# dzatulin/llama-fastapi-k8s-gpu

Measured on AMD Instinct MI355X. Metric: output tokens/sec + p50 /response latency, Llama-3-8B Q4_K_M at 1/2/4/8 MI355X, higher is better.
Workload: dtype q4_k_m weights; f16 (batched decode and prompt prefill MFMA, tile16 copies) / int8 (single-row GEMV) activations; fp32 accumulate

## Files before the change

csrc/bindings_hip.cpp:

```cpp
#include <pybind11/functional.h>
#include <pybind11/numpy.h>
#include <pybind11/pybind11.h>
#include <pybind11/stl.h>

#include <array>
#include <rccl/rccl.h>

#include "bind_scheduler.h"
#include "kernels/kernels.h"
#include "runtime/engine.h"
#include "runtime/repack.h"

namespace py = pybind11;
using namespace lfk;

template <class T>
static T* P(uintptr_t p) { return reinterpret_cast<T*>(p); }
static hipStream_t S(uintptr_t s) { return reinterpret_cast<hipStream_t>(s); }

static void hip_ok(const char* what) {
  hipError_t e = hipGetLastError();
  if (e != hipSuccess) throw std::runtime_error(std::string(what) + ": " + hipGetErrorString(e));
}

// ... 305 lines not shown
  });

  m.def("bprep", [](uintptr_t x, int ldx, bool swiglu, uintptr_t norm, float eps, int K, int B, uintptr_t xh, int ldh,
                    uintptr_t stream, uintptr_t zero, int zero_n, int swiglu_group) {
    BPrepArgs a;
    a.swiglu_group = swiglu_group;
    a.x = P<float>(x); a.ldx = ldx; a.swiglu = swiglu; a.norm_w = P<float>(norm); a.eps = eps; a.K = K; a.B = B;
    a.xh = P<__half>(xh); a.ldh = ldh; a.zero = P<float>(zero); a.zero_n = zero_n;
    bprep(a, S(stream));
    hip_ok("bprep");
  }, py::arg("x"), py::arg("ldx"), py::arg("swiglu"), py::arg("norm"), py::arg("eps"), py::arg("K"), py::arg("B"),
     py::arg("xh"), py::arg("ldh"), py::arg("stream"), py::arg("zero") = 0, py::arg("zero_n") = 0,
     py::arg("swiglu_group") = 32);
  m.def("bmm", [](uintptr_t w, int type, int rows, int K, uintptr_t xh, int ldh, uintptr_t out, int ldo, int B,
                  uintptr_t stream, int debug, uintptr_t h_out, int ldh_out, uintptr_t xf, int ldxf,
                  uintptr_t norm, float eps, bool store_out, uintptr_t dbg_clk, int tr) {
    BmmArgs a;
    a.debug = debug;
    a.tr = tr;
    a.dbg_clk = P<long long>(dbg_clk);
    a.w = make_qmat(P<void>(w), type, rows, K);
    a.xh = P<__half>(xh); a.ldh = ldh; a.out = P<float>(out); a.ldo = ldo; a.n_out = rows; a.B = B;
    if (h_out) {
      a.swiglu_epi = true; a.h_out = P<__half>(h_out); a.ldh_out = ldh_out;
    }
    if (xf) {
      a.xf = P<float>(xf); a.ldxf = ldxf; a.norm_w = P<float>(norm); a.eps = eps;
    }
    a.store_out = store_out;
    bmm(a, S(stream));
    hip_ok("bmm");
  }, py::arg("w"), py::arg("type"), py::arg("rows"), py::arg("K"), py::arg("xh"), py::arg("ldh"), py::arg("out"),
     py::arg("ldo"), py::arg("B"), py::arg("stream"), py::arg("debug") = 0, py::arg("h_out") = 0,
     py::arg("ldh_out") = 0, py::arg("xf") = 0, py::arg("ldxf") = 0, py::arg("norm") = 0, py::arg("eps") = 1e-5f,
     py::arg("store_out") = false, py::arg("dbg_clk") = 0, py::arg("tr") = -1);
  m.def("chain_layout", []() { return std::make_tuple(kChainStride, kChainXcds, kChainInts); });
  m.def("bmm_ffn_chain", [](uintptr_t wg, int tg, int F, int K, uintptr_t xh, uintptr_t xf, uintptr_t norm, float eps,
                            uintptr_t wd, int td, uintptr_t hout, uintptr_t out, int B, uintptr_t cnt,
                            uintptr_t stream, int tr) {
    BmmArgs gu, dn;
    dn.tr = tr;
    gu.w = make_qmat(P<void>(wg), tg, 2 * F, K);
    gu.xh = P<__half>(xh); gu.ldh = K; gu.n_out = 2 * F; gu.B = B;
    gu.swiglu_epi = true; gu.h_out = P<__half>(hout); gu.ldh_out = F;
    if (xf) {
      gu.xf = P<float>(xf); gu.ldxf = K; gu.norm_w = P<float>(norm); gu.eps = eps;
    }
    dn.w = make_qmat(P<void>(wd), td, K, F);
    dn.xh = P<__half>(hout); dn.ldh = F; dn.out = P<float>(out); dn.ldo = K; dn.n_out = K; dn.B = B;
    if (!bmm_ffn_chain_supported(gu, dn)) throw std::runtime_error("bmm_ffn_chain: unsupported shapes");
    bmm_ffn_chain(gu, dn, P<int>(cnt), nullptr, S(stream));
    hip_ok("bmm_ffn_chain");
  }, py::arg("wg"), py::arg("tg"), py::arg("F"), py::arg("K"), py::arg("xh"), py::arg("xf"), py::arg("norm"),
     py::arg("eps"), py::arg("wd"), py::arg("td"), py::arg("hout"), py::arg("out"), py::arg("B"), py::arg("cnt"),
     py::arg("stream"), py::arg("tr") = -1);
  m.def("bmm_wo_ffn_chain", [](uintptr_t wo, int to, int Kwo, uintptr_t xa, uintptr_t wg, int tg, int F, int K,
                               uintptr_t norm, float eps, uintptr_t wd, int td, uintptr_t xh, uintptr_t hout,
                               uintptr_t resid, int B, uintptr_t cnt, uintptr_t stream, int tr) {
    BmmArgs o, gu, dn;
    o.tr = dn.tr = tr;
    o.w = make_qmat(P<void>(wo), to, K, Kwo);
    o.xh = P<__half>(xa); o.ldh = Kwo; o.out = P<float>(resid); o.ldo = K; o.n_out = K; o.B = B;
    gu.w = make_qmat(P<void>(wg), tg, 2 * F, K);
    gu.xh = P<__half>(xh); gu.ldh = K; gu.n_out = 2 * F; gu.B = B;
    gu.swiglu_epi = true; gu.h_out = P<__half>(hout); gu.ldh_out = F;
    gu.xf = P<float>(resid); gu.ldxf = K; gu.norm_w = P<float>(norm); gu.eps = eps;
    dn.w = make_qmat(P<void>(wd), td, K, F);
    dn.xh = P<__half>(hout); dn.ldh = F; dn.out = P<float>(resid); dn.ldo = K; dn.n_out = K; dn.B = B;
    if (!bmm_wo_ffn_chain_supported(o, gu, dn)) throw std::runtime_error("bmm_wo_ffn_chain: unsupported shapes");
    bmm_wo_ffn_chain(o, gu, dn, P<int>(cnt), nullptr, S(stream));
// ... 273 lines not shown
```

csrc/kernels/bmm.hip:

```cpp
#include <algorithm>
#include <cstdlib>
#include <stdexcept>

#include "gemv_dev.h"

namespace lfk {

typedef _Float16 h2_t __attribute__((ext_vector_type(2)));
typedef _Float16 h8_t __attribute__((ext_vector_type(8)));
typedef float f4_t __attribute__((ext_vector_type(4)));

__device__ __forceinline__ h2_t as_h2(unsigned v) { return __builtin_bit_cast(h2_t, v); }
__device__ __forceinline__ unsigned as_u(h2_t v) { return __builtin_bit_cast(unsigned, v); }

__device__ __forceinline__ unsigned bytes02(unsigned x) { return __builtin_amdgcn_perm(0x64646464u, x, 0x04020400u); }
__device__ __forceinline__ unsigned bytes13(unsigned x) { return __builtin_amdgcn_perm(0x64646464u, x, 0x04030401u); }

__device__ __forceinline__ unsigned deq_pair(unsigned magic_pair, h2_t bias, h2_t a, h2_t m) {
  const h2_t v = as_h2(magic_pair) - bias;
  return as_u(v * a + m);
}

struct HFrag {
  unsigned w[16];
// ... 778 lines not shown
      const float ss = wave_sum_fast(x.x * x.x + x.y * x.y + x.z * x.z + x.w * x.w);
      if (lane == 0) atomicAdd(rowss + b, ss);
    }
  }
}

template <int N>
using f32v = float __attribute__((ext_vector_type(N)));
template <int N>
using u32v = unsigned __attribute__((ext_vector_type(N)));
__device__ __forceinline__ float4 ldg4(const float* p) {
  typedef float v4 __attribute__((ext_vector_type(4)));
  const v4 t = *(const __attribute__((address_space(1))) v4*)(p);
  return make_float4(t.x, t.y, t.z, t.w);
}
__device__ __forceinline__ uint4 ldg4(const __half* p) {
  typedef unsigned v4 __attribute__((ext_vector_type(4)));
  const v4 t = *(const __attribute__((address_space(1))) v4*)(p);
  return make_uint4(t.x, t.y, t.z, t.w);
}
template <int N>
__device__ __forceinline__ void vput(f32v<N>& v, int i, float4 t) {
  v[4 * i] = t.x; v[4 * i + 1] = t.y; v[4 * i + 2] = t.z; v[4 * i + 3] = t.w;
}
template <int N>
__device__ __forceinline__ float4 vget(const f32v<N>& v, int i) {
  return make_float4(v[4 * i], v[4 * i + 1], v[4 * i + 2], v[4 * i + 3]);
}
template <int NW, bool SC1 = false, class Issue>
__device__ __forceinline__ void xfirst_norm(const BmmArgs& a, __half* xs, float* rowss, int ldx, int tid, int lane,
// ... 174 lines not shown
  }();
  return a.tr < 0 ? v : a.tr != 0;
}

template <int QT, int PD, bool SK, int NW = 8, bool MOE = false, bool XF = false, int DBG = 0, bool IL = false,
          int EPI = 0, int CR = 0, bool TR = false>
__device__ __forceinline__ void wt_body(const BmmArgs& a, const int run, const int bid, const int nblk) {
  constexpr int R = PD + 1;
  extern __shared__ __attribute__((aligned(16))) char smem[];
  float* rowss = reinterpret_cast<float*>(smem);
  __half* xs = reinterpret_cast<__half*>(smem + 256);
  {
    const int f0 = a.w.K, f1 = a.kparts, f2 = a.spp, f3 = a.n_out, f4 = a.B, f5 = a.nseg, f6 = a.debug, f7 = a.chain_role;
    const int f8 = a.ldh, f9 = a.ldxf, f10 = a.zero_n, f11 = a.ldo, f12 = a.nb1, f13 = a.tpg, f14 = a.seg_split;
    const void *p0 = a.w.base, *p1 = a.xh, *p2 = a.xf, *p3 = a.norm_w, *p4 = a.zero, *p5 = a.dbg_clk, *p6 = a.out,
               *p7 = a.chain_cnt, *p8 = a.ss_out;
    asm volatile("" ::"s"(f0), "s"(f1), "s"(f2), "s"(f3), "s"(f4), "s"(f5), "s"(f6), "s"(f7), "s"(f8), "s"(f9), "s"(f10),
                 "s"(f11), "s"(f12), "s"(f13), "s"(f14), "s"(p0), "s"(p1), "s"(p2), "s"(p3), "s"(p4), "s"(p5), "s"(p6),
                 "s"(p7), "s"(p8), "s"(nblk));
  }
  const int lane = threadIdx.x & 63, wave = wave_id(), tid = threadIdx.x;
  const int r16 = lane & 15, kq = lane >> 4;
  const int K = a.w.K, steps = K >> 8;
  const int kparts = a.kparts, kp = bid % kparts, grp = bid / kparts, G = nblk / kparts;
  const int s0 = kp * a.spp, ns = min(steps, s0 + a.spp) - s0;
  const int k0 = s0 * 256, kn = ns * 256, ldx = kn + kWtXPad;
  if (MOE && !SK && a.ew && a.steps_per_expert > 0) {
    const int e = s0 / a.steps_per_expert;
    bool any = false;
    for (int b = 0; b < a.B; ++b) any = any || a.ew[(size_t)b * a.ew_ld + e] != 0.f;
    if (!any) {
      if (a.zero) {
        float4* z = reinterpret_cast<float4*>(a.zero);
        for (int i = bid * (NW * 64) + threadIdx.x; i < (a.zero_n >> 2); i += nblk * (NW * 64))
// ... 107 lines not shown
    for (int p = 0; p < PD; ++p) load_first(buf[p], p < N);
    if constexpr (SK && !IL) pos = a.qkv.pos[col_ok ? r16 : 0];
    if (!XF && xmode == 2) lds_barrier();
  };
  if (XF && xmode == 2) lds_barrier();
  __shared__ int wo_exits;
  if (tid == 0) wo_exits = 0;
  auto wo_arrive = [&]() {
    if (!SK && (a.chain_role & kChainWoDone)) {
      asm volatile("s_waitcnt vmcnt(0)" ::: "memory");
      if (lane == 0 && atomicAdd(&wo_exits, 1) == NW - 1)
        __hip_atomic_fetch_add(a.chain_cnt + (kChainWoPart * kChainXcds + (xcc_id() & (kChainXcds - 1))) * kChainStride, 1,
                               __ATOMIC_RELAXED, __HIP_MEMORY_SCOPE_AGENT);
    }
  };
  if constexpr (DBG == 4 || DBG == 6) issue();
  else if constexpr (XF) {
    if constexpr (!SK && CR == kChainConsume) {
      issue();
      chain_wait(a, kp, tid);
      xstage_sc1<NW>(a, xs, ldx, k0, kn, tid);
    } else if constexpr (!SK && CR == kChainWaitWo) {
      issue();
      count_wait(a, kChainWoPart, a.chain_wo, tid);
      xfirst_norm<NW, true>(a, xs, rowss, ldx, tid, lane, wave, [] {});
    } else if (xmode == 2) xfirst_part_norm<NW>(a, xs, rowss, ldx, k0, kn, tid, lane, issue);
    else if (xmode == 1) xfirst_norm<NW>(a, xs, rowss, ldx, tid, lane, wave, issue);
    else xfirst_plain<NW>(a, xs, rowss, ldx, k0, kn, tid, lane, wave, issue);
  } else {
    issue();
    if (xmode == 2) stage_x_part_norm<NW>(a, xs, rowss, ldx, k0, kn, tid, lane);
    else bmm_stage_x<NW>(a, xs, rowss, ldx, k0, kn, tid, lane, wave);
  }
  if constexpr (XF) lds_barrier();
  else __syncthreads();
  if (clk && tid == 0) clk[2] = wall_clock64();
  if (!SK && (a.chain_role & kChainProduce) && tid == 0)
    __hip_atomic_fetch_add(a.chain_cnt + (kChainStagedPart * kChainXcds + (xcc_id() & (kChainXcds - 1))) * kChainStride, 1,
                           __ATOMIC_RELAXED, __HIP_MEMORY_SCOPE_AGENT);
  if (SK && a.ss_out && run == 0 && grp == 0 && tid < a.B) atomicAdd(a.ss_out + tid, rowss[tid]);
  if (N == 0) {
    wo_arrive();
    return;
  }
  if constexpr (SK && !IL) {
    pos = min(max(pos, 0), a.qkv.n_ctx - 1);
    rope_load(0);
  }
  float cs = 1.f;
  if (a.xf && !SK) {
    float t = 0.f;
#pragma unroll
    for (int w = 0; w < NW; ++w) t += rowss[(col_ok ? r16 : 0) * NW + w];
    cs = rsqrtf(t / (float)K + a.eps);
  }
  const __half* xrow = xs + (col_ok ? r16 : 0) * ldx - k0;
  f4_t acc = {0.f, 0.f, 0.f, 0.f}, acc2 = {0.f, 0.f, 0.f, 0.f};
  int ci = 0, cstep = 0;
  auto add_tr = [&](float* o, int row0, int n_out, bool atomic) {
    if (row0 + r16 < n_out) {
#pragma unroll
      for (int i = 0; i < 4; ++i) {
        const int b = 4 * kq + i;
        if (b < a.B) {
          float* p = o + (size_t)b * a.ldo + row0 + r16;
// ... 1 lines not shown
          else if (a.store_out) *p = acc[i];
          else *p += acc[i];
        }
      }
    }
  };
  auto finish = [&]() {
    acc += acc2;
    if (a.debug == 3) {
      asm volatile("" ::"v"(acc[0]), "v"(acc[1]), "v"(acc[2]), "v"(acc[3]));
      acc = f4_t{0.f, 0.f, 0.f, 0.f};
      acc2 = acc;
      return;
    }
    if constexpr (!TR) {
      if (a.xf && !SK) acc *= cs;
    }
    const int gt = tile_of(ci);
    if constexpr (SK) {
      const int sg = seg_of(gt), kind = sg == 0 ? a.qkv.kind[0] : sg == 1 ? a.qkv.kind[1] : a.qkv.kind[2];
      const int n_out = sg == 0 ? a.n_out : sg == 1 ? a.seg_rows[1] : a.seg_rows[2];
      float* o = (sg == 0 ? a.out : sg == 1 ? a.seg_out[1] : a.seg_out[2]) + (size_t)r16 * a.ldo;
      const int row0 = (gt - seg_first(sg)) * 16 + 4 * kq;
      f4_t y = acc;
      if (!IL && kind < 2) {
#pragma unroll
        for (int j = 0; j < 2; ++j) {
          y[2 * j] = acc[2 * j] * rc[j].x - acc[2 * j + 1] * rc[j].y;
          y[2 * j + 1] = acc[2 * j] * rc[j].y + acc[2 * j + 1] * rc[j].x;
        }
      }
// ... 147 lines not shown
  (void)a;
  (void)b;
}

template <int QT0, int QT1, int QT2, bool TR = false>
__global__ __launch_bounds__(512, 2) void bmm_chain3_kernel(BmmArgs a, BmmArgs b, BmmArgs c) {
  const BmmArgs* ka = (const BmmArgs*)__builtin_amdgcn_kernarg_segment_ptr();
  const int n0 = ka[0].nb1, n1 = ka[1].nb1;
  const int bid = blockIdx.x;
  if (bid < n0) wt_body<QT0, 2, false, 8, false, true, 0, true, 2, 0, TR>(ka[0], 0, bid, n0);
  else if (bid < n0 + n1) wt_body<QT1, 2, false, 8, false, true, 0, true, 1, kChainWaitWo>(ka[1], 0, bid - n0, n1);
  else wt_body<QT2, 2, false, 8, false, true, 0, true, 2, kChainConsume, TR>(ka[2], 0, bid - n0 - n1, gridDim.x - n0 - n1);
  (void)a;
  (void)b;
  (void)c;
}

static constexpr int kPrepBlock = 1024;
static constexpr int kPrepMaxVec = 8;

__global__ __launch_bounds__(kPrepBlock) void bprep_kernel(BPrepArgs a) {
  __shared__ float red[kPrepBlock / 64];
  const int b = blockIdx.x, tid = threadIdx.x;
  if (b >= a.B) {
    float4* z = reinterpret_cast<float4*>(a.zero);
    const int nzb = gridDim.x - a.B;
    for (int i = (b - a.B) * kPrepBlock + tid; i < (a.zero_n >> 2); i += nzb * kPrepBlock)
      z[i] = make_float4(0.f, 0.f, 0.f, 0.f);
    return;
  }
// ... 240 lines not shown
  if (a.ew && (a.ew_ld < 1 || (a.swiglu_epi ? a.tiles_per_expert < 1 || ((a.n_out + 15) / 16) % a.tiles_per_expert
                                            : a.steps_per_expert < 1 || (a.w.K / 256) % a.steps_per_expert)))
    throw std::runtime_error("bmm: expert routing weights need whole experts of tiles / K steps");
  if (a.ew && a.swiglu_epi && (a.n_out + 15) / 16 / a.tiles_per_expert > 64) throw std::runtime_error("bmm: <= 64 experts");
  if (a.ew && !a.swiglu_epi && (a.xf || a.qkv_epi || a.one_part))
    throw std::runtime_error("bmm: the MoE down projection runs split-K (whole-expert parts)");
  if (a.qkv_sk) {
    if (a.B > 8 || a.qkv_epi || a.swiglu_epi || a.ew || a.one_part || a.store_out || !a.qkv.pos || !a.qkv.rope ||
        a.qkv.head_dim % 2 || a.qkv.n_ctx < 1 || a.seg_split < 1 || a.seg_split > a.nseg ||
        (a.seg_split < a.nseg && !bmm_qkv_sk_supported(a.w.type, a.type2, a.type2, a.w.K, a.B)))
      throw std::runtime_error("bmm: split-K Q|K|V arguments");
    if (a.xf && (!a.norm_w || !a.ss_out || a.ldxf < a.w.K || a.ldxf % 4)) throw std::runtime_error("bmm: split-K Q|K|V norm");
  }
  if (a.ss_out && !(a.qkv_sk && a.xf)) throw std::runtime_error("bmm: ss_out needs the split-K Q|K|V norm");
  if (a.zero && (a.zero_n % 4 || reinterpret_cast<uintptr_t>(a.zero) % 16)) throw std::runtime_error("bmm: zero side job alignment");
}

void bmm(const BmmArgs& a0, hipStream_t s) {
  BmmArgs a = a0;
  bmm_check(a);
  if (a.n_out <= 0) return;
  a.w.type = t16_kernel_type(a.w.type);
  a.type2 = a.type2 ? t16_kernel_type(a.type2) : 0;
  if (a.qkv_sk && a.seg_split < a.nseg && a.type2 == a.w.type) {
    a.seg_split = a.nseg;
    a.type2 = 0;
  }
  if (a.qkv_sk) {
    const bool two = a.seg_split < a.nseg;
    const int t2 = two ? a.type2 : 0;
// ... 71 lines not shown
  if (dn.kparts > kChainWoPart) throw std::runtime_error("bmm_wo_ffn_chain: too many K parts for the counters");
  wo.chain_role = kChainWoDone; wo.chain_cnt = cnt; wo.nb1 = n0;
  gu.chain_role = kChainProduce | kChainWaitWo; gu.chain_cnt = cnt; gu.chain_tpp = 32 * dn.spp; gu.chain_wo = n0;
  gu.chain_err = err; gu.chain_poll = 8; gu.nb1 = n1;
  dn.chain_role = kChainConsume; dn.chain_cnt = cnt; dn.chain_tpp = 32 * dn.spp; dn.chain_tiles = (gu.n_out + 15) / 16;
  dn.chain_err = err; dn.chain_staged = n1; dn.chain_poll = 8;
  const dim3 grid(n0 + n1 + n2);
  const size_t lds = std::max(lds0, std::max(lds1, lds2));
  if (bmm_tr(dn)) {
    if (dn.w.type == T_Q6_K) hipLaunchKernelGGL((bmm_chain3_kernel<T_Q4_K, T_Q4_K, T_Q6_K, true>), grid, dim3(512), lds, s, wo, gu, dn);
    else hipLaunchKernelGGL((bmm_chain3_kernel<T_Q4_K, T_Q4_K, T_Q4_K, true>), grid, dim3(512), lds, s, wo, gu, dn);
  } else if (dn.w.type == T_Q6_K) hipLaunchKernelGGL((bmm_chain3_kernel<T_Q4_K, T_Q4_K, T_Q6_K>), grid, dim3(512), lds, s, wo, gu, dn);
  else hipLaunchKernelGGL((bmm_chain3_kernel<T_Q4_K, T_Q4_K, T_Q4_K>), grid, dim3(512), lds, s, wo, gu, dn);
}

bool bmm_qkv2(const BmmArgs& a0, const BmmArgs& b0, hipStream_t s) {
  if (!a0.qkv_epi || !b0.qkv_epi || a0.B != b0.B || a0.w.K != b0.w.K || a0.n_out <= 0 || b0.n_out <= 0)
    return false;
  if ((a0.xf == nullptr) != (b0.xf == nullptr)) return false;
  BmmArgs a = a0, b = b0;
  bmm_check(a);
  bmm_check(b);
  auto tiles_of = [](const BmmArgs& x) {
    int t = (x.n_out + 15) / 16;
    for (int i = 1; i < x.nseg; ++i) t += (x.seg_rows[i] + 15) / 16;
    return t;
  };
  const int steps = a.w.K / 256;
  a.spp = b.spp = steps;
  a.kparts = b.kparts = 1;
// ... 294 lines not shown
```

csrc/kernels/kernels.h:

```cpp
#pragma once
#include <hip/hip_bf16.h>
#include <hip/hip_fp16.h>
#include <hip/hip_runtime.h>

#include <cstddef>
#include <cstdint>

#include "../common.h"

namespace lfk {

struct QMat {
  const uint8_t* base = nullptr;
  int type = 0;
  int rows = 0;
  int K = 0;
  Planes P{};
  size_t expert_stride = 0;
};

QMat make_qmat(const void* base, int type, int rows, int K, size_t expert_stride = 0);

inline size_t qmat_bytes(const QMat& m) {
  const size_t R = (size_t)m.rows;
// ... 94 lines not shown
    int n_ctx = 0, head_dim = 0;
    const int* pos = nullptr;
    const int* slots = nullptr;
    const float2* rope = nullptr;
    const float* bias[3] = {nullptr, nullptr, nullptr};
  } qkv;
  bool qkv_epi = false;
  __half* h_out = nullptr;
  int ldh_out = 0;
  bool swiglu_epi = false;
  int tile_groups = 1;
  const float* xf = nullptr;
  int ldxf = 0;
  const float* norm_w = nullptr;
  float eps = 1e-5f;
  bool store_out = false;
  const float* ew = nullptr;
  int ew_ld = 0, tiles_per_expert = 0, steps_per_expert = 0;
  bool one_part = false;
  int tr = -1;
  long long* dbg_clk = nullptr;
  int nb1 = 0;
  bool qkv_sk = false;
  float* ss_out = nullptr;
  int seg_split = 1;
  int type2 = 0;
  int tpg = 8;
  float* zero = nullptr;
  int zero_n = 0;
};
bool bmm_qkv_sk_supported(int tq, int tk, int tv, int K, int B);
bool bmm_supported(int type, int K);
bool bmm_qkv_fits(int K, int B);
bool bmm_norm_fits(int K, int B);
void bmm(const BmmArgs& a, hipStream_t s);
constexpr int kChainStride = 32, kChainXcds = 8, kChainMaxParts = 16;
constexpr int kChainInts = kChainStride * kChainXcds * kChainMaxParts;
constexpr int kChainStagedPart = kChainMaxParts - 1;
constexpr int kChainWoPart = kChainMaxParts - 2;
constexpr int kChainProduce = 1, kChainConsume = 2, kChainWoDone = 4, kChainWaitWo = 8;
bool bmm_ffn_chain_supported(const BmmArgs& gu, const BmmArgs& dn);
void bmm_ffn_chain(const BmmArgs& gu, const BmmArgs& dn, int* cnt, int* err, hipStream_t s);
bool bmm_wo_ffn_chain_supported(const BmmArgs& wo, const BmmArgs& gu, const BmmArgs& dn);
void bmm_wo_ffn_chain(const BmmArgs& wo, const BmmArgs& gu, const BmmArgs& dn, int* cnt, int* err, hipStream_t s);
bool bmm_qkv2(const BmmArgs& a, const BmmArgs& b, hipStream_t s);
bool bmm_qkv_sk_defers_rope();
size_t t16_bytes(int type, int rows, int K);
int t16_format(int type);
void t16_repack(const QMat& planar, uint8_t* dst, hipStream_t s, bool swiglu = false);
struct BPrepArgs {
  const float* x = nullptr;
  int ldx = 0;
  bool swiglu = false;
  const float* norm_w = nullptr;
  float eps = 1e-5f;
  int K = 0, B = 0;
  __half* xh = nullptr;
  int ldh = 0;
  float* zero = nullptr;
// ... 215 lines not shown
```

csrc/runtime/engine.cpp:

```cpp
#include "engine.h"

#include <rccl/rccl.h>
#include <rocprofiler-sdk-roctx/roctx.h>

#include <chrono>
#include <cmath>
#include <cstdio>
#include <cstring>
#include <stdexcept>

#include "repack.h"
#include "shard.h"

namespace lfk {

#define HIPCHK(x) check((x), #x)

struct RoctxRange {
  explicit RoctxRange(const char* m) { roctxRangePushA(m); }
  ~RoctxRange() { roctxRangePop(); }
};

static double now_s() {
  return std::chrono::duration<double>(std::chrono::steady_clock::now().time_since_epoch()).count();
// ... 418 lines not shown
    chain_cnt_ = (int*)dalloc(sizeof(int) * kChainInts * hp_.n_layer);
    HIPCHK(hipMemsetAsync(chain_cnt_, 0, sizeof(int) * kChainInts * hp_.n_layer, stream_));
    HIPCHK(hipHostMalloc((void**)&chain_err_h_, sizeof(int), hipHostMallocMapped));
    *chain_err_h_ = 0;
    HIPCHK(hipHostGetDevicePointer((void**)&chain_err_, chain_err_h_, 0));
  }
  const int E = std::max(1, hp_.n_expert);
  xh_b_ = (__half*)dalloc(2ull * bmax_ * std::max({hp_.n_embd, nq_, F_l_}));
  {
    const size_t n = qkv_b_zero_n();
    qkv_b_ = (float*)dalloc(sizeof(float) * n);
    HIPCHK(hipMemsetAsync(qkv_b_, 0, sizeof(float) * n, stream_));
    ss_b_ = qkv_b_ + (size_t)bmax_ * (nq_ + 2 * nkvd_);
  }
  hh_b_ = (__half*)dalloc(2ull * bmax_ * std::max(1, F_l_) * (moe_b_ ? E : 1));
  if (moe_b_) ew_b_ = (float*)dalloc(sizeof(float) * bmax_ * E);
  auto tile = [&](const QMat& m, bool swiglu = false) {
    QMat t = m;
    uint8_t* dst = (uint8_t*)dalloc(t16_bytes(m.type, m.rows, m.K));
    t16_repack(m, dst, stream_, swiglu);
    t.base = dst;
    return t;
  };
  t_output_ = tile(output_);
  for (int l = 0; l < hp_.n_layer; ++l) {
    Layer& L = layers_[l];
    L.t_wq = tile(L.wq); L.t_wk = tile(L.wk); L.t_wv = tile(L.wv); L.t_wo = tile(L.wo);
    if (bg_ffn_) { L.t_gu = tile(L.w_gu, true); L.t_down = tile(L.w_down); }
    if (moe_b_) {
      const size_t gu1 = t16_bytes(L.gu_exps.type, L.gu_exps.rows, L.gu_exps.K);
// ... 665 lines not shown
  };
  auto tp_end = [&]() {
    if (tp_acc) p2p_->allreduce_add(tmp_b_, x_, B * d, s);
    else if (tp) allreduce_into(tmp_, x_, (size_t)B * d, s);
  };
  const size_t kv_layer = (size_t)nkv_l_ * opt_.n_ctx * hd;
  __half* kcl = kc_ + kv_layer * (l - opt_.layer_begin);
  __half* vcl = vc_ + kv_layer * (l - opt_.layer_begin);
  const bool fused = B <= kBmmMaxRows && bmm_qkv_fits(d, B);
  const bool fnorm = fused && bmm_norm_fits(d, B);
  const bool sk = qkv_sk_ && bmm_qkv_sk_supported(L.t_wq.type, L.t_wk.type, L.t_wv.type, d, B) &&
                  (!L.bqkv || bmm_qkv_sk_defers_rope());
  auto zero_qkv = [&]() {
    if (sk) HIPCHK(hipMemsetAsync(qkv_b_, 0, sizeof(float) * qkv_b_zero_n(), s));
  };
  if (sk) {
    BmmArgs a;
    a.w = L.t_wq; a.n_out = L.t_wq.rows; a.out = qkv_b_; a.ldo = ncol; a.B = B;
    a.nseg = 3;
    a.seg_base[1] = L.t_wk.base; a.seg_rows[1] = L.t_wk.rows; a.seg_out[1] = qkv_b_ + nq_;
    a.seg_base[2] = L.t_wv.base; a.seg_rows[2] = L.t_wv.rows; a.seg_out[2] = qkv_b_ + nq_ + nkvd_;
    const int tq = t16_format(L.t_wq.type), tk = t16_format(L.t_wk.type), tv = t16_format(L.t_wv.type);
    a.seg_split = tk != tq ? 1 : tv != tq ? 2 : 3;
    a.type2 = tk != tq ? tk : tv != tq ? tv : 0;
    a.qkv_sk = true;
    a.qkv.pos = bpos_; a.qkv.rope = rope_; a.qkv.head_dim = hd; a.qkv.n_ctx = opt_.n_ctx;
    a.xf = x_; a.ldxf = d; a.norm_w = L.attn_norm; a.eps = hp_.rms_eps; a.ss_out = ss_b_;
    a.dbg_clk = clk_of(l, 0);
    bmm(a, s);
  } else {
// ... 45 lines not shown
  aa.scale = 1.f / std::sqrt((float)hd);
  aa.part = attn_part_b_; aa.counters = attn_cnt_b_; aa.out = attn_;
  aa.batch = B; aa.slots = bslots_; aa.slot_stride = slot_stride_;
  aa.q_stride = nq_; aa.out_stride = nq_;
  aa.part_stride = attn_decode_workspace_floats(opt_.n_ctx, nh_l_, hd);
  aa.out_h = xh_b_; aa.out_h_stride = nq_;
  aa.out = nullptr;
  if (sk) {
    aa.qkv_raw = qkv_b_; aa.qkv_ld = ncol; aa.k_off = nq_; aa.v_off = nq_ + nkvd_;
    aa.ss = ss_b_; aa.inv_k = 1.f / (float)d; aa.eps = hp_.rms_eps;
    if (bmm_qkv_sk_defers_rope()) aa.rope_freq = rope_freq_;
    aa.qkv_bias = L.bqkv;
  }
  aa.dbg_clk = clk_of(l, 1);
  attn_decode(aa, s);
  BmmArgs wo, gu, dn;
  wo.w = L.t_wo; wo.xh = xh_b_; wo.ldh = nq_; wo.out = acc; wo.ldo = d; wo.n_out = d; wo.B = B;
  wo.dbg_clk = clk_of(l, 2);
  const bool dense_ffn = !(moe_b_ && fused) && bg_ffn_ && fused;
  if (dense_ffn) {
    if (fnorm) {
      gu.xf = x_; gu.ldxf = d; gu.norm_w = L.ffn_norm; gu.eps = hp_.rms_eps;
    }
    gu.w = L.t_gu; gu.xh = xh_b_; gu.ldh = d;
    gu.out = nullptr; gu.ldo = 0; gu.n_out = 2 * F_l_; gu.B = B;
    gu.swiglu_epi = true; gu.h_out = hh_b_; gu.ldh_out = F_l_;
    gu.dbg_clk = clk_of(l, 3);
    dn.w = L.t_down; dn.xh = hh_b_; dn.ldh = F_l_; dn.out = acc; dn.ldo = d; dn.n_out = d; dn.B = B;
    dn.dbg_clk = clk_of(l, 4);
    if (sk) {
      dn.zero = qkv_b_; dn.zero_n = (int)qkv_b_zero_n();
    }
    if (ffn_chain_ >= 2 && !tp && fnorm && B <= kBmmMaxRows && bmm_wo_ffn_chain_supported(wo, gu, dn)) {
      bmm_wo_ffn_chain(wo, gu, dn, chain_cnt_ + kChainInts * l, chain_err_, s);
      return;
    }
  }
  tp_begin();
  if (B <= kBmmMaxRows) bmm(wo, s);
  else bmm_rows(L.t_wo, xh_b_, nq_, acc, d, d, B, s, clk_of(l, 2));
  tp_end();
  if (moe_b_ && fused) {
    const int E = hp_.n_expert;
    moe_router_rows(x_, d, B, L.ffn_norm, hp_.rms_eps, reinterpret_cast<const float*>(L.router.base), d, E,
                    hp_.n_expert_used, ew_b_, E, s);
    BmmArgs a;
    if (fnorm) {
      a.xf = x_; a.ldxf = d; a.norm_w = L.ffn_norm; a.eps = hp_.rms_eps;
    } else {
      bprep_rows(x_, d, false, L.ffn_norm, d, B, nullptr, 0, s);
    }
    a.w = L.t_gu; a.xh = xh_b_; a.ldh = d;
    a.out = nullptr; a.ldo = 0; a.n_out = L.t_gu.rows; a.B = B;
    a.swiglu_epi = true; a.h_out = hh_b_; a.ldh_out = E * F_l_;
// ... 954 lines not shown
```

csrc/runtime/engine.h:

```cpp
#pragma once
#include <hip/hip_runtime.h>

#include <atomic>
#include <functional>
#include <memory>
#include <mutex>
#include <string>
#include <vector>

#include "../kernels/kernels.h"
#include "gguf.h"
#include "p2p.h"
#include "slots.h"
#include "tp_channel.h"

namespace lfk {


struct EngineOptions {
  int n_ctx = 1024;
  int n_batch = 512;
  int device = 0;
  bool use_graph = true;
  int tp_rank = 0;
// ... 269 lines not shown
  long long* step_clk_ = nullptr;
  int step_clk_layer_ = -1;
  long long* clk_of(int l, int k) const {
    return l == step_clk_layer_ && step_clk_ ? step_clk_ + (size_t)k * kStepClkBlocks * 16 : nullptr;
  }
  float* qkv_b_ = nullptr;
  float* ss_b_ = nullptr;
  bool wo_fuse_ = true;
  bool moe_route_fuse_ = true;
  int* wo_err_h_ = nullptr;
  int* wo_err_ = nullptr;
  int ffn_chain_ = 1;
  int* chain_cnt_ = nullptr;
  int* chain_err_h_ = nullptr;
  int* chain_err_ = nullptr;
  int* dec_done_ = nullptr;
  size_t qkv_b_zero_n() const { return (size_t)bmax_ * (nq_ + 2 * nkvd_) + 16; }

  std::vector<hipGraphExec_t> bgraph_;
  std::vector<hipGraphExec_t> bgraph2_;
  int launch_par_ = 0;
  int dslot_ = 0;
  std::vector<hipGraphExec_t> sgraph_, sgraph2_;
  bool last_b1_ = false;
  hipGraph_t graph_ = nullptr;
  hipGraphExec_t graph_exec_ = nullptr, graph_exec2_ = nullptr;
  void enqueue_stage_decode(hipStream_t s);
  void chain_step(const Engine* prev, const Engine* last, const std::vector<Engine*>& others);
  hipGraphExec_t chain_graph_[2] = {nullptr, nullptr};
  int chain_par_ = 0;
// ... 7 lines not shown
```

Measured before the change: 2860.

## Fuse FFN RMSNorm prep into a wave-owned Wo kernel with deferred row scale

Adds a Wo projection kernel in which each block owns a 16-column tile over the full K. It adds the residual, writes the updated residual, emits the norm-weighted f16 FFN input and per-tile partial sums of squares. The gate/up SwiGLU kernel then reads those f16 rows and reduces the partial sums to apply the RMS scale after accumulation, instead of staging and normalising fp32 rows itself. This is meant to remove the per-block norm/staging work in gate/up for small decode batches (B<=8). The cost is that Wo runs with only n_out/16 blocks and no split-K, and the activation is rounded to f16 before the scale is applied.

Result: no change. 2858 (-0.0%).

```diff
diff --git a/csrc/bindings_hip.cpp b/csrc/bindings_hip.cpp
--- a/csrc/bindings_hip.cpp
+++ b/csrc/bindings_hip.cpp
@@ -343,7 +343,7 @@
      py::arg("swiglu_group") = 32);
   m.def("bmm", [](uintptr_t w, int type, int rows, int K, uintptr_t xh, int ldh, uintptr_t out, int ldo, int B,
                   uintptr_t stream, int debug, uintptr_t h_out, int ldh_out, uintptr_t xf, int ldxf,
-                  uintptr_t norm, float eps, bool store_out, uintptr_t dbg_clk, int tr) {
+                  uintptr_t norm, float eps, bool store_out, uintptr_t dbg_clk, int tr, uintptr_t xss) {
     BmmArgs a;
     a.debug = debug;
     a.tr = tr;
@@ -356,17 +356,41 @@
     if (xf) {
       a.xf = P<float>(xf); a.ldxf = ldxf; a.norm_w = P<float>(norm); a.eps = eps;
     }
+    if (xss) {
+      a.xss = P<float>(xss); a.eps = eps;
+    }
     a.store_out = store_out;
     bmm(a, S(stream));
     hip_ok("bmm");
   }, py::arg("w"), py::arg("type"), py::arg("rows"), py::arg("K"), py::arg("xh"), py::arg("ldh"), py::arg("out"),
      py::arg("ldo"), py::arg("B"), py::arg("stream"), py::arg("debug") = 0, py::arg("h_out") = 0,
      py::arg("ldh_out") = 0, py::arg("xf") = 0, py::arg("ldxf") = 0, py::arg("norm") = 0, py::arg("eps") = 1e-5f,
-     py::arg("store_out") = false, py::arg("dbg_clk") = 0, py::arg("tr") = -1);
+     py::arg("store_out") = false, py::arg("dbg_clk") = 0, py::arg("tr") = -1, py::arg("xss") = 0);
+  m.def("bmm_wo_own", [](uintptr_t w, int type, int rows, int K, uintptr_t xh, int ldh, uintptr_t out, int ldo, int B,
+                         uintptr_t norm, uintptr_t hn, int ldhn, uintptr_t ss, uintptr_t stream, uintptr_t dbg_clk) {
+    BmmArgs a;
+    a.w = make_qmat(P<void>(w), type, rows, K);
+    a.xh = P<__half>(xh); a.ldh = ldh; a.out = P<float>(out); a.ldo = ldo; a.n_out = rows; a.B = B;
+    a.norm_w = P<float>(norm); a.h_out = P<__half>(hn); a.ldh_out = ldhn; a.ss_out = P<float>(ss);
+    a.dbg_clk = P<long long>(dbg_clk);
+    bmm_wo_own(a, S(stream));
+    hip_ok("bmm_wo_own");
+  }, py::arg("w"), py::arg("type"), py::arg("rows"), py::arg("K"), py::arg("xh"), py::arg("ldh"), py::arg("out"),
+     py::arg("ldo"), py::arg("B"), py::arg("norm"), py::arg("hn"), py::arg("ldhn"), py::arg("ss"), py::arg("stream"),
+     py::arg("dbg_clk") = 0);
+  m.def("bmm_wo_own_supported", [](int type, int rows, int K, int B) {
+    BmmArgs a;
+    __half* h = reinterpret_cast<__half*>(16);
+    float* f = reinterpret_cast<float*>(16);
+    a.w = make_qmat(nullptr, type, rows, K);
+    a.xh = h; a.ldh = K; a.out = f; a.ldo = rows; a.n_out = rows; a.B = B; a.norm_w = f; a.h_out = h; a.ldh_out = rows;
+    a.ss_out = f;
+    return bmm_wo_own_supported(a);
+  });
   m.def("chain_layout", []() { return std::make_tuple(kChainStride, kChainXcds, kChainInts); });
   m.def("bmm_ffn_chain", [](uintptr_t wg, int tg, int F, int K, uintptr_t xh, uintptr_t xf, uintptr_t norm, float eps,
                             uintptr_t wd, int td, uintptr_t hout, uintptr_t out, int B, uintptr_t cnt,
-                            uintptr_t stream, int tr) {
+                            uintptr_t stream, int tr, uintptr_t xss) {
     BmmArgs gu, dn;
     dn.tr = tr;
     gu.w = make_qmat(P<void>(wg), tg, 2 * F, K);
@@ -375,6 +399,9 @@
     if (xf) {
       gu.xf = P<float>(xf); gu.ldxf = K; gu.norm_w = P<float>(norm); gu.eps = eps;
     }
+    if (xss) {
+      gu.xss = P<float>(xss); gu.eps = eps;
+    }
     dn.w = make_qmat(P<void>(wd), td, K, F);
     dn.xh = P<__half>(hout); dn.ldh = F; dn.out = P<float>(out); dn.ldo = K; dn.n_out = K; dn.B = B;
     if (!bmm_ffn_chain_supported(gu, dn)) throw std::runtime_error("bmm_ffn_chain: unsupported shapes");
@@ -382,7 +409,7 @@
     hip_ok("bmm_ffn_chain");
   }, py::arg("wg"), py::arg("tg"), py::arg("F"), py::arg("K"), py::arg("xh"), py::arg("xf"), py::arg("norm"),
      py::arg("eps"), py::arg("wd"), py::arg("td"), py::arg("hout"), py::arg("out"), py::arg("B"), py::arg("cnt"),
-     py::arg("stream"), py::arg("tr") = -1);
+     py::arg("stream"), py::arg("tr") = -1, py::arg("xss") = 0);
   m.def("bmm_wo_ffn_chain", [](uintptr_t wo, int to, int Kwo, uintptr_t xa, uintptr_t wg, int tg, int F, int K,
                                uintptr_t norm, float eps, uintptr_t wd, int td, uintptr_t xh, uintptr_t hout,
                                uintptr_t resid, int B, uintptr_t cnt, uintptr_t stream, int tr) {
diff --git a/csrc/kernels/bmm.hip b/csrc/kernels/bmm.hip
--- a/csrc/kernels/bmm.hip
+++ b/csrc/kernels/bmm.hip
@@ -816,6 +816,7 @@
   const v4 t = *(const __attribute__((address_space(1))) v4*)(p);
   return make_float4(t.x, t.y, t.z, t.w);
 }
+__device__ __forceinline__ float ldg1(const float* p) { return *(const __attribute__((address_space(1))) float*)(p); }
 __device__ __forceinline__ uint4 ldg4(const __half* p) {
   typedef unsigned v4 __attribute__((ext_vector_type(4)));
   const v4 t = *(const __attribute__((address_space(1))) v4*)(p);
@@ -1020,10 +1021,10 @@
     const int f0 = a.w.K, f1 = a.kparts, f2 = a.spp, f3 = a.n_out, f4 = a.B, f5 = a.nseg, f6 = a.debug, f7 = a.chain_role;
     const int f8 = a.ldh, f9 = a.ldxf, f10 = a.zero_n, f11 = a.ldo, f12 = a.nb1, f13 = a.tpg, f14 = a.seg_split;
     const void *p0 = a.w.base, *p1 = a.xh, *p2 = a.xf, *p3 = a.norm_w, *p4 = a.zero, *p5 = a.dbg_clk, *p6 = a.out,
-               *p7 = a.chain_cnt, *p8 = a.ss_out;
+               *p7 = a.chain_cnt, *p8 = a.ss_out, *p9 = a.xss;
     asm volatile("" ::"s"(f0), "s"(f1), "s"(f2), "s"(f3), "s"(f4), "s"(f5), "s"(f6), "s"(f7), "s"(f8), "s"(f9), "s"(f10),
                  "s"(f11), "s"(f12), "s"(f13), "s"(f14), "s"(p0), "s"(p1), "s"(p2), "s"(p3), "s"(p4), "s"(p5), "s"(p6),
-                 "s"(p7), "s"(p8), "s"(nblk));
+                 "s"(p7), "s"(p8), "s"(p9), "s"(nblk));
   }
   const int lane = threadIdx.x & 63, wave = wave_id(), tid = threadIdx.x;
   const int r16 = lane & 15, kq = lane >> 4;
@@ -1161,6 +1162,12 @@
                                __ATOMIC_RELAXED, __HIP_MEMORY_SCOPE_AGENT);
     }
   };
+  constexpr bool XSS = !SK && !TR && NW == 8 && (EPI == 0 || EPI == 1);
+  f4_t xssv = {0.f, 0.f, 0.f, 0.f};
+  if constexpr (XSS) {
+    const float4 t = ldg4(a.xss ? a.xss + min(tid >> 1, (K >> 4) - 1) * 8 + 4 * (tid & 1) : reinterpret_cast<const float*>(a.w.base));
+    xssv = f4_t{t.x, t.y, t.z, t.w};
+  }
   if constexpr (DBG == 4 || DBG == 6) issue();
   else if constexpr (XF) {
     if constexpr (!SK && CR == kChainConsume) {
@@ -1179,6 +1186,20 @@
     if (xmode == 2) stage_x_part_norm<NW>(a, xs, rowss, ldx, k0, kn, tid, lane);
     else bmm_stage_x<NW>(a, xs, rowss, ldx, k0, kn, tid, lane, wave);
   }
+  if constexpr (XSS) {
+    if (a.xss) {
+      if ((tid >> 1) >= (K >> 4)) xssv = f4_t{0.f, 0.f, 0.f, 0.f};
+#pragma unroll
+      for (int m = 2; m < 64; m <<= 1) {
+#pragma unroll
+        for (int c = 0; c < 4; ++c) xssv[c] += __shfl_xor(xssv[c], m);
+      }
+      if (lane < 2) {
+#pragma unroll
+        for (int c = 0; c < 4; ++c) rowss[(4 * lane + c) * NW + wave] = xssv[c];
+      }
+    }
+  }
   if constexpr (XF) lds_barrier();
   else __syncthreads();
   if (clk && tid == 0) clk[2] = wall_clock64();
@@ -1195,7 +1216,7 @@
     rope_load(0);
   }
   float cs = 1.f;
-  if (a.xf && !SK) {
+  if (!SK && (a.xf || (XSS && a.xss))) {
     float t = 0.f;
 #pragma unroll
     for (int w = 0; w < NW; ++w) t += rowss[(col_ok ? r16 : 0) * NW + w];
@@ -1227,7 +1248,7 @@
       return;
     }
     if constexpr (!TR) {
-      if (a.xf && !SK) acc *= cs;
+      if ((a.xf || (XSS && a.xss)) && !SK) acc *= cs;
     }
     const int gt = tile_of(ci);
     if constexpr (SK) {
@@ -1405,6 +1426,92 @@
   (void)a;
   (void)b;
   (void)c;
+}
+
+template <int QT>
+__global__ __launch_bounds__(512, 2) void bmm_wo_own_kernel(BmmArgs a_) {
+  const BmmArgs& a = *(const BmmArgs*)__builtin_amdgcn_kernarg_segment_ptr();
+  constexpr int NW = 8;
+  extern __shared__ __attribute__((aligned(16))) char smem[];
+  float* red = reinterpret_cast<float*>(smem);
+  __half* xs = reinterpret_cast<__half*>(smem + (NW - 1) * 64 * 16);
+  {
+    const int f0 = a.w.K, f1 = a.spp, f2 = a.B, f3 = a.ldh, f4 = a.ldo, f5 = a.ldh_out;
+    const void *p0 = a.w.base, *p1 = a.xh, *p2 = a.out, *p3 = a.norm_w, *p4 = a.h_out, *p5 = a.ss_out, *p6 = a.dbg_clk;
+    asm volatile("" ::"s"(f0), "s"(f1), "s"(f2), "s"(f3), "s"(f4), "s"(f5), "s"(p0), "s"(p1), "s"(p2), "s"(p3), "s"(p4),
+                 "s"(p5), "s"(p6));
+  }
+  const int lane = threadIdx.x & 63, wave = wave_id(), tid = threadIdx.x;
+  const int r16 = lane & 15, kq = lane >> 4;
+  const int K = a.w.K, steps = K >> 8, ldx = K + kWtXPad, B = a.B;
+  const int tile = blockIdx.x, col = tile * 16 + r16;
+  const int ws0 = wave * a.spp, wn = max(0, min(a.spp, steps - ws0));
+  constexpr int SB = t16_step_bytes(QT);
+  long long* clk = a.dbg_clk ? a.dbg_clk + (size_t)tile * 8 : nullptr;
+  if (clk && tid == 0) {
+    clk[0] = wall_clock64();
+    clk[6] = xcc_id();
+  }
+  auto rsrc = [](const uint8_t* p) { return __builtin_amdgcn_make_buffer_rsrc(const_cast<uint8_t*>(p), 0, 0x7FFFFFFF, 0x00020000); };
+  const auto rs_tile = rsrc(a.w.base + (size_t)tile * steps * SB), rs0 = rsrc(a.w.base);
+  BRawT<QT> b0[2], b1[2];
+  auto load = [&](BRawT<QT>* dst, int s, bool real) {
+    const auto rs = real ? rs_tile : rs0;
+    const int so = real ? s * SB : 0;
+    tload_rs<QT>(dst[0], rs, so, 0, lane, r16, kq);
+    tload_rs<QT>(dst[1], rs, so, 1, lane, r16, kq);
+  };
+  f4_t res;
+  float nw;
+  auto issue = [&]() __attribute__((always_inline)) {
+    if (clk && tid == 0) clk[1] = wall_clock64();
+    load(b0, ws0, wn > 0);
+    load(b1, ws0 + 1, wn > 1);
+#pragma unroll
+    for (int i = 0; i < 4; ++i) res[i] = ldg1(a.out + (size_t)min(4 * kq + i, B - 1) * a.ldo + col);
+    nw = ldg1(a.norm_w + col);
+  };
+  xfirst_plain<NW>(a, xs, nullptr, ldx, 0, K, tid, lane, wave, issue);
+  lds_barrier();
+  if (clk && tid == 0) clk[2] = wall_clock64();
+  const __half* xrow = xs + (r16 < B ? r16 : 0) * ldx;
+  f4_t acc = {0.f, 0.f, 0.f, 0.f}, acc2 = {0.f, 0.f, 0.f, 0.f};
+  if (wn > 0) bmm_step<QT, false, true, true>(b0, ws0, kq, xrow, acc, acc2);
+  if (wn > 1) bmm_step<QT, false, true, true>(b1, ws0 + 1, kq, xrow, acc, acc2);
+  for (int j = 2; j < wn; j += 2) {
+    load(b0, ws0 + j, true);
+    load(b1, ws0 + j + 1, j + 1 < wn);
+    bmm_step<QT, false, true, true>(b0, ws0 + j, kq, xrow, acc, acc2);
+    if (j + 1 < wn) bmm_step<QT, false, true, true>(b1, ws0 + j + 1, kq, xrow, acc, acc2);
+  }
+  acc += acc2;
+  if (wave > 0) *reinterpret_cast<f4_t*>(red + ((wave - 1) * 64 + lane) * 4) = acc;
+  lds_barrier();
+  if (wave != 0) return;
+  if (clk && tid == 0) clk[3] = wall_clock64();
+#pragma unroll
+  for (int w = 0; w < NW - 1; ++w) acc += *reinterpret_cast<const f4_t*>(red + (w * 64 + lane) * 4);
+  const int hcol = (col & ~3) | ((col & 1) << 1) | ((col >> 1) & 1);
+#pragma unroll
+  for (int i = 0; i < 4; ++i) {
+    const int b = 4 * kq + i;
+    const float x = res[i] + acc[i];
+    if (b < B) {
+      a.out[(size_t)b * a.ldo + col] = x;
+      a.h_out[(size_t)b * a.ldh_out + hcol] = __float2half(x * nw);
+    }
+    float ss = x * x;
+    ss += __shfl_xor(ss, 1);
+    ss += __shfl_xor(ss, 2);
+    ss += __shfl_xor(ss, 4);
+    ss += __shfl_xor(ss, 8);
+    if (b < B && r16 == 0) a.ss_out[tile * 8 + b] = ss;
+  }
+  if (clk && tid == 0) {
+    clk[4] = wall_clock64();
+    clk[5] = 1;
+  }
+  (void)a_;
 }
 
 static constexpr int kPrepBlock = 1024;
@@ -1675,6 +1782,8 @@
   }
   if (a.ss_out && !(a.qkv_sk && a.xf)) throw std::runtime_error("bmm: ss_out needs the split-K Q|K|V norm");
   if (a.zero && (a.zero_n % 4 || reinterpret_cast<uintptr_t>(a.zero) % 16)) throw std::runtime_error("bmm: zero side job alignment");
+  if (a.xss && (!a.swiglu_epi || a.xf || a.ew || a.B > 8 || !a.xh || a.w.K > 4096))
+    throw std::runtime_error("bmm: the deferred row scale runs in the wave-owned SwiGLU gate/up (B <= 8, K <= 4096, f16 rows)");
 }
 
 void bmm(const BmmArgs& a0, hipStream_t s) {
@@ -1776,6 +1885,34 @@
   else hipLaunchKernelGGL((bmm_chain3_kernel<T_Q4_K, T_Q4_K, T_Q4_K>), grid, dim3(512), lds, s, wo, gu, dn);
 }
 
+static size_t wo_own_lds(int K, int B) { return (size_t)7 * 64 * 16 + (size_t)B * (K + kWtXPad) * 2; }
+
+bool bmm_wo_own_supported(const BmmArgs& a) {
+  return bmm_supported(a.w.type, a.w.K) && a.B >= 1 && a.B <= 8 && a.n_out > 0 && a.n_out % 16 == 0 &&
+         a.n_out / 16 <= bmm_cus() && wo_own_lds(a.w.K, a.B) <= 150 * 1024 && a.nseg == 1 && !a.ew && !a.xf && !a.xss &&
+         !a.swiglu_epi && !a.qkv_epi && !a.qkv_sk && !a.one_part && !a.store_out && !a.zero && !a.chain_role && !a.debug &&
+         a.xh && a.ldh >= a.w.K && a.ldh % 8 == 0 && a.out && a.ldo >= a.n_out && a.norm_w && a.h_out && a.ss_out &&
+         a.ldh_out >= a.n_out;
+}
+
+void bmm_wo_own(const BmmArgs& a0, hipStream_t s) {
+  if (!bmm_wo_own_supported(a0)) throw std::runtime_error("bmm_wo_own: unsupported shape");
+  BmmArgs a = a0;
+  a.w.type = t16_kernel_type(a.w.type);
+  const int steps = a.w.K / 256;
+  a.kparts = 1;
+  a.spp = (steps + 7) / 8;
+  const size_t lds = std::max<size_t>(wo_own_lds(a.w.K, a.B), 81 * 1024);
+  const dim3 grid(a.n_out / 16);
+  switch (a.w.type) {
+    case T_Q4_K: hipLaunchKernelGGL((bmm_wo_own_kernel<T_Q4_K>), grid, dim3(512), lds, s, a); break;
+    case T_Q5_K: hipLaunchKernelGGL((bmm_wo_own_kernel<T_Q5_K>), grid, dim3(512), lds, s, a); break;
+    case T_Q6_K: hipLaunchKernelGGL((bmm_wo_own_kernel<T_Q6_K>), grid, dim3(512), lds, s, a); break;
+    case T_Q8_0: hipLaunchKernelGGL((bmm_wo_own_kernel<T_Q8_0>), grid, dim3(512), lds, s, a); break;
+    default: throw std::runtime_error("bmm_wo_own: unsupported weight type");
+  }
+}
+
 bool bmm_qkv2(const BmmArgs& a0, const BmmArgs& b0, hipStream_t s) {
   if (!a0.qkv_epi || !b0.qkv_epi || a0.B != b0.B || a0.w.K != b0.w.K || a0.n_out <= 0 || b0.n_out <= 0)
     return false;
diff --git a/csrc/kernels/kernels.h b/csrc/kernels/kernels.h
--- a/csrc/kernels/kernels.h
+++ b/csrc/kernels/kernels.h
@@ -132,6 +132,7 @@
   int ldxf = 0;
   const float* norm_w = nullptr;
   float eps = 1e-5f;
+  const float* xss = nullptr;
   bool store_out = false;
   const float* ew = nullptr;
   int ew_ld = 0, tiles_per_expert = 0, steps_per_expert = 0;
@@ -161,6 +162,8 @@
 void bmm_ffn_chain(const BmmArgs& gu, const BmmArgs& dn, int* cnt, int* err, hipStream_t s);
 bool bmm_wo_ffn_chain_supported(const BmmArgs& wo, const BmmArgs& gu, const BmmArgs& dn);
 void bmm_wo_ffn_chain(const BmmArgs& wo, const BmmArgs& gu, const BmmArgs& dn, int* cnt, int* err, hipStream_t s);
+bool bmm_wo_own_supported(const BmmArgs& a);
+void bmm_wo_own(const BmmArgs& a, hipStream_t s);
 bool bmm_qkv2(const BmmArgs& a, const BmmArgs& b, hipStream_t s);
 bool bmm_qkv_sk_defers_rope();
 size_t t16_bytes(int type, int rows, int K);
diff --git a/csrc/runtime/engine.cpp b/csrc/runtime/engine.cpp
--- a/csrc/runtime/engine.cpp
+++ b/csrc/runtime/engine.cpp
@@ -456,6 +456,11 @@
     ss_b_ = qkv_b_ + (size_t)bmax_ * (nq_ + 2 * nkvd_);
   }
   hh_b_ = (__half*)dalloc(2ull * bmax_ * std::max(1, F_l_) * (moe_b_ ? E : 1));
+  if (const char* e = std::getenv("LFK_WO_OWN")) wo_own_ = e[0] != '0';
+  if (wo_own_) {
+    xn_b_ = (__half*)dalloc(2ull * bmax_ * hp_.n_embd);
+    xss_b_ = (float*)dalloc(sizeof(float) * 8 * ((hp_.n_embd + 15) / 16));
+  }
   if (moe_b_) ew_b_ = (float*)dalloc(sizeof(float) * bmax_ * E);
   auto tile = [&](const QMat& m, bool swiglu = false) {
     QMat t = m;
@@ -1151,6 +1156,13 @@
   auto zero_qkv = [&]() {
     if (sk) HIPCHK(hipMemsetAsync(qkv_b_, 0, sizeof(float) * qkv_b_zero_n(), s));
   };
+  BmmArgs wo, wown;
+  wo.w = L.t_wo; wo.xh = xh_b_; wo.ldh = nq_; wo.out = acc; wo.ldo = d; wo.n_out = d; wo.B = B;
+  wo.dbg_clk = clk_of(l, 2);
+  wown = wo;
+  wown.norm_w = L.ffn_norm; wown.h_out = xn_b_; wown.ldh_out = d; wown.ss_out = xss_b_;
+  const bool own = wo_own_ && sk && !tp && fnorm && bg_ffn_ && !moe_b_ && ffn_chain_ < 2 && B <= 8 &&
+                   bmm_wo_own_supported(wown);
   if (sk) {
     BmmArgs a;
     a.w = L.t_wq; a.n_out = L.t_wq.rows; a.out = qkv_b_; a.ldo = ncol; a.B = B;
@@ -1226,15 +1238,16 @@
   }
   aa.dbg_clk = clk_of(l, 1);
   attn_decode(aa, s);
-  BmmArgs wo, gu, dn;
-  wo.w = L.t_wo; wo.xh = xh_b_; wo.ldh = nq_; wo.out = acc; wo.ldo = d; wo.n_out = d; wo.B = B;
-  wo.dbg_clk = clk_of(l, 2);
+  BmmArgs gu, dn;
   const bool dense_ffn = !(moe_b_ && fused) && bg_ffn_ && fused;
   if (dense_ffn) {
     if (fnorm) {
       gu.xf = x_; gu.ldxf = d; gu.norm_w = L.ffn_norm; gu.eps = hp_.rms_eps;
     }
     gu.w = L.t_gu; gu.xh = xh_b_; gu.ldh = d;
+    if (own) {
+      gu.xf = nullptr; gu.norm_w = nullptr; gu.xh = xn_b_; gu.xss = xss_b_;
+    }
     gu.out = nullptr; gu.ldo = 0; gu.n_out = 2 * F_l_; gu.B = B;
     gu.swiglu_epi = true; gu.h_out = hh_b_; gu.ldh_out = F_l_;
     gu.dbg_clk = clk_of(l, 3);
@@ -1249,7 +1262,8 @@
     }
   }
   tp_begin();
-  if (B <= kBmmMaxRows) bmm(wo, s);
+  if (own) bmm_wo_own(wown, s);
+  else if (B <= kBmmMaxRows) bmm(wo, s);
   else bmm_rows(L.t_wo, xh_b_, nq_, acc, d, d, B, s, clk_of(l, 2));
   tp_end();
   if (moe_b_ && fused) {
diff --git a/csrc/runtime/engine.h b/csrc/runtime/engine.h
--- a/csrc/runtime/engine.h
+++ b/csrc/runtime/engine.h
@@ -307,6 +307,9 @@
   int* chain_cnt_ = nullptr;
   int* chain_err_h_ = nullptr;
   int* chain_err_ = nullptr;
+  bool wo_own_ = true;
+  __half* xn_b_ = nullptr;
+  float* xss_b_ = nullptr;
   int* dec_done_ = nullptr;
   size_t qkv_b_zero_n() const { return (size_t)bmax_ * (nq_ + 2 * nkvd_) + 16; }
 
```
